# NTV-UIT/MARLLB

Hardware: AMD Instinct MI355X
Metric: env-steps/sec (whole node), 4-server LB env, batch 4k→512k at 1/2/4/8 MI355X (higher is better)
Workload: dtype fp32/int32 (f64 reward); 1 GPU; LB env random-policy rollout, 4 servers (BASELINE configs[1] rollout at the north-star batch); assign_policy=sed, envs_per_gpu=65536, servers=4, global_batch=65536, autoreset=True, autoreset_mode=same_step, parallelism=env-shard x1, dyn_mapping=auto

## Files before the change

### marllb_amd/csrc/lbsim_dyn_group.h

```cpp
#pragma once

#include "lbsim_cross.h"
#include "lbsim_delay.h"
#include "lbsim_kernels.h"
#include "lbsim_workers.h"

namespace lbk {

constexpr int kGroupWL = 8;

template <int CTRL>
__device__ __forceinline__ uint32_t gdpp(uint32_t v) {
  return (uint32_t)__builtin_amdgcn_mov_dpp((int)v, CTRL, 0xF, 0xF, true);
}
__device__ __forceinline__ int32_t f32_key(float x) {
  const int32_t b = (int32_t)__float_as_uint(x);
  return b ^ ((b >> 31) & 0x7FFFFFFF);
}
__device__ __forceinline__ float key_f32(int32_t k) {
  return __uint_as_float((uint32_t)(k ^ ((k >> 31) & 0x7FFFFFFF)));
}
template <int CTRL>
__device__ __forceinline__ void gmin_step(int32_t& a, int32_t& b) {
  const int32_t oa = (int32_t)gdpp<CTRL>((uint32_t)a);
  const int32_t ob = (int32_t)gdpp<CTRL>((uint32_t)b);
  a = oa < a ? oa : a;
  b = ob < b ? ob : b;
}
template <int G>
__device__ __forceinline__ void group_min2(int32_t& a, int32_t& b) {
  gmin_step<0xB1>(a, b);
  if constexpr (G >= 4) gmin_step<0x4E>(a, b);
  if constexpr (G >= 8) gmin_step<0x141>(a, b);
  if constexpr (G >= 16) gmin_step<0x140>(a, b);
  if constexpr (G >= 32) {
    int32_t oa = __shfl_xor(a, 16, 64), ob = __shfl_xor(b, 16, 64);
    a = oa < a ? oa : a;
    b = ob < b ? ob : b;
    if constexpr (G >= 64) {
      oa = __shfl_xor(a, 32, 64);
      ob = __shfl_xor(b, 32, 64);
      a = oa < a ? oa : a;
      b = ob < b ? ob : b;
    }
  }
}
template <int G>
__device__ __forceinline__ int32_t group_min_i32(int32_t v) {
  int32_t o = (int32_t)gdpp<0xB1>((uint32_t)v);
  v = o < v ? o : v;
  if constexpr (G >= 4) { o = (int32_t)gdpp<0x4E>((uint32_t)v); v = o < v ? o : v; }
  if constexpr (G >= 8) { o = (int32_t)gdpp<0x141>((uint32_t)v); v = o < v ? o : v; }
  if constexpr (G >= 16) { o = (int32_t)gdpp<0x140>((uint32_t)v); v = o < v ? o : v; }
  if constexpr (G >= 32) { o = __shfl_xor(v, 16, 64); v = o < v ? o : v; }
  if constexpr (G >= 64) { o = __shfl_xor(v, 32, 64); v = o < v ? o : v; }
  return v;
}
template <int G>
__device__ __forceinline__ uint32_t group_add(uint32_t v) {
  v += gdpp<0xB1>(v);
  if constexpr (G >= 4) v += gdpp<0x4E>(v);
  if constexpr (G >= 8) v += gdpp<0x141>(v);
  if constexpr (G >= 16) v += gdpp<0x140>(v);
  if constexpr (G >= 32) v += (uint32_t)__shfl_xor((int)v, 16, 64);
  if constexpr (G >= 64) v += (uint32_t)__shfl_xor((int)v, 32, 64);
  return v;
}
template <int G>
__device__ __forceinline__ uint32_t group_or(uint32_t v) {
  v |= gdpp<0xB1>(v);
  if constexpr (G >= 4) v |= gdpp<0x4E>(v);
  if constexpr (G >= 8) v |= gdpp<0x141>(v);
  if constexpr (G >= 16) v |= gdpp<0x140>(v);
  if constexpr (G >= 32) v |= (uint32_t)__shfl_xor((int)v, 16, 64);
  if constexpr (G >= 64) v |= (uint32_t)__shfl_xor((int)v, 32, 64);
  return v;
}
template <int G>
__device__ __forceinline__ uint64_t group_bits(uint64_t m, int gbase) {
  return G == 64 ? m : (m >> gbase) & ((1ull << (G & 63)) - 1ull);
}

struct SrvLane {
  int32_t cnt, head_tc, head, lh, tail, last, assigned;
  int32_t qcap;
  bool big;
  uint32_t rcnt;
  int32_t lost;
  uint32_t* chgw;
  float score, scale;
  double den, rcp;
  bool act;
  uint32_t rcnt_d;
  int32_t phead, pcnt;
  uint32_t pdue, over;
  uint32_t* fs_row;
  uint32_t fs_cnt, fs_max;
  unsigned long long fs_sum;
};

__device__ __forceinline__ void flow_stats_add(SrvLane& V, uint32_t fct) {
  if (V.fs_row == nullptr) return;
  V.fs_cnt += 1u;
  V.fs_sum += fct;
  V.fs_max = fct > V.fs_max ? fct : V.fs_max;
  V.fs_row[flow_bin(fct)] += 1u;
}

struct CrossLane {
  bool on = false;
  uint32_t thr = 0u, edge = 0u, salt = 0u;
};

struct WorkLane {
  bool on = false;
  int32_t c = 1;
};

struct DelayLane {
  bool pend = false;
  int32_t r = 0;
  float w2 = 1.0f;
};

struct LaneQueue {
  int2* win;
  int2* ring;
  int lane, lh, head, Q;
  __device__ __forceinline__ int2 get(int pos) const {
    int2 e;
    if (workers_in_window(pos, kGroupWL)) {
      e = win[workers_win_slot(lh, pos, kGroupWL) * 64 + lane];
    } else {
      e = ring[(uint32_t)workers_ring_index(head, pos, Q)];
      asm volatile("");
    }
    return e;
  }
  __device__ __forceinline__ void set(int pos, const int2& e) const {
    if (workers_in_window(pos, kGroupWL)) {
      win[workers_win_slot(lh, pos, kGroupWL) * 64 + lane] = e;
    } else {
      ring[(uint32_t)workers_ring_index(head, pos, Q)] = e;
      asm volatile("");
    }
  }
};

struct GroupAliasTab {
  int32_t* t;
  int gbase;
  __device__ int32_t& operator()(int f, int k) const { return t[f * 64 + gbase + k]; }
};

__device__ __forceinline__ void split_add(const DevState& st, const SimParams& p, SrvLane& V,
                                          uint32_t sb, uint32_t gid, uint32_t episode, int s,
                                          bool is_dur, uint32_t v, uint32_t ts_ms, bool has_r,
                                          uint32_t r) {
  const uint32_t c = is_dur ? V.rcnt_d : V.rcnt;
  const int slot = res_slot(p, c, has_r, r, gid, episode,
                            (kStreamReservoir << 24) | (is_dur ? 0u : 1u << 16) | (uint32_t)s);
  if (slot >= 0) {
    if (!has_r && v >= kPackLimit) V.big = true;
    uint2* rec = is_dur ? reinterpret_cast<uint2*>(st.res_dur) : st.res;
    rec[(size_t)sb * K + (uint32_t)slot] = make_uint2(v, ts_ms);
    atomicOr(V.chgw + ((uint32_t)slot >> 5) * 64u, 1u << (slot & 31));
  }
  if (is_dur) V.rcnt_d = count_inc(c);
  else V.rcnt = count_inc(c);
}
__device__ __forceinline__ void split_flush(const DevState& st, const SimParams& p, SrvLane& V,
                                            uint32_t sb, uint32_t gid, uint32_t episode, int s,
                                            int32_t t, uint64_t base_us) {
  const int P = p.pend_P;
  const uint2* ring = st.pend + (size_t)sb * (uint32_t)P;
  while (V.pcnt > 0) {
    const int32_t rel = (int32_t)(V.pdue - (uint32_t)base_us);
    if (rel > t) break;
    const uint32_t val = ring[V.phead].y;
    const uint32_t ts = (uint32_t)((uint64_t)((int64_t)base_us + (int64_t)rel) / 1000u);
    split_add(st, p, V, sb, gid, episode, s, false, val, ts, false, 0u);
    V.phead = V.phead + 1 == P ? 0 : V.phead + 1;
    V.pcnt -= 1;
    if (V.pcnt > 0) V.pdue = ring[V.phead].x;
  }
}
__device__ __forceinline__ void split_push(const DevState& st, const SimParams& p, SrvLane& V,
                                           uint32_t sb, uint32_t due, uint32_t val) {
  const int P = p.pend_P;
  if (V.pcnt == P) {
    V.over += 1u;
    return;
  }
  uint2* ring = st.pend + (size_t)sb * (uint32_t)P;
  int i = V.pcnt;
  while (i > 0) {
    int pos = V.phead + i - 1;
    pos = pos >= P ? pos - P : pos;
    const uint2 e = ring[pos];
    if ((int32_t)(e.x - due) <= 0) break;
    ring[pos + 1 == P ? 0 : pos + 1] = e;
    --i;
  }
  int pos = V.phead + i;
  pos = pos >= P ? pos - P : pos;
  ring[pos] = make_uint2(due, val);
  V.pcnt += 1;
  if (i == 0) V.pdue = due;
}
__device__ __forceinline__ void split_complete(const DevState& st, const SimParams& p, SrvLane& V,
                                               uint32_t sb, uint32_t gid, uint32_t episode, int s,
                                               int32_t tc, int32_t ta, uint32_t dur, uint32_t ts_ms,
                                               bool has_r, uint32_t r, uint64_t base_us) {
  split_flush(st, p, V, sb, gid, episode, s, tc, base_us);
  split_add(st, p, V, sb, gid, episode, s, true, dur, ts_ms, has_r, r);
  int32_t wait = 0;
  if (lf_wait(p, (uint32_t)base_us + (uint32_t)ta, gid, episode, wait))
    split_push(st, p, V, sb,
               (uint32_t)base_us + (uint32_t)tc + (uint32_t)(p.lf_off_us + 40000000) +
                   (uint32_t)wait,
               lf_guess((uint32_t)(tc - ta), p.lf_off_us, wait));
  else
    split_add(st, p, V, sb, gid, episode, s, false, (uint32_t)(tc - ta), ts_ms, has_r, r);
}
__device__ __forceinline__ void vpp_zero_bins(const DevState& st, const SimParams& p, uint32_t sb) {
  uint4* r4 = reinterpret_cast<uint4*>(st.res + (size_t)sb * K);
  for (int i = 0; i < K / 2; ++i) r4[i] = make_uint4(0u, 0u, 0u, 0u);
  if (st.res_dur != nullptr) {
    const int n4 = p.split ? K / 2 : K / 4;
    uint4* d4 = reinterpret_cast<uint4*>(st.res_dur + (size_t)sb * K * (p.split ? 2u : 1u));
    for (int i = 0; i < n4; ++i) d4[i] = make_uint4(0u, 0u, 0u, 0u);
  }
}

struct GroupConst {
  uint32_t k0, k1;
  float mean_gap;
  int32_t dt;
  uint32_t base_ms, base_rem;
};
__device__ __forceinline__ GroupConst group_const(const SimParams& p, float mean_gap,
                                                  uint32_t base_ms, uint32_t base_rem) {
  GroupConst c;
  c.k0 = vpin(p.key0);
  c.k1 = vpin(p.key1);
  c.mean_gap = vpin(mean_gap);
  c.dt = vpin(p.dt_us);
  c.base_ms = vpin(base_ms);
  c.base_rem = vpin(base_rem);
  return c;
}

template <int G, int POLICY, bool TRACE, bool FAST, bool FULL = false, bool DELAY = false>
__device__ __forceinline__ void group_event_loop(const DevState& st, const SimParams& p,
                                                 LaneState<1>& E, SrvLane& V, int s, int gbase,
                                                 int n_alias, const GroupConst& gc, int2* win,
                                                 int32_t* atab, int4* acache, uint2* const my_res,
                                                 int2* const my_ring, bool fs_on = false,
                                                 const TraceSel& ts = TraceSel{},
                                                 const WorkSel& ws = WorkSel{},
                                                 const CrossLane& cx = CrossLane{},
                                                 const WorkLane& wk = WorkLane{},
                                                 DelayLane dl = DelayLane{}) {
  constexpr int WL = kGroupWL;
  constexpr bool two_choice = (POLICY == 1 || POLICY == 3);
  constexpr bool alias = POLICY == kPolicyAlias;
  constexpr bool lsq = (POLICY == 2 || POLICY == 3);
  const int S = p.S, Q = p.Q;
  const int32_t dt = gc.dt;
  const GroupAliasTab tab{atab, gbase};
  const int lane = gbase + s;
  auto wslot = [&](int i) -> int2* { return win + i * 64 + lane; };
  auto mark = [&](int slot) {
    atomicOr(V.chgw + ((uint32_t)slot >> 5) * 64u, 1u << (slot & 31));
  };
  uint32_t cbase = 0u;
  uint32_t it = 0u;
  uint32_t kbase = E.arr_idx + 1u, rbase = 0u;
  if constexpr (TRACE) rbase = trace_row_in(ts.rows, E.gid, E.episode, kbase);
  for (;;) {
    if constexpr (DELAY && !lsq) {
      if (dl.pend && E.next_arr >= dl.r) {
        dl.pend = false;
        if constexpr (alias) {
          const float w2 = dl.w2;
          n_alias = build_alias_fn<G>([&](int k) { return __shfl(w2, gbase + k, 64); }, S, tab);
        } else if (V.act) {
          V.den = (double)dl.w2 + 1e-9;
          V.rcp = 1.0 / V.den;
        }
      }
    }
    if ((it & (uint32_t)(G - 1)) == 0u) {
      cbase = E.arr_idx + 1u;
      const uint32_t k = cbase + (uint32_t)s;
      uint32_t rk0[10], rk1[10];
      const uint32_t k0 = gc.k0, k1 = gc.k1;
#pragma unroll
      for (int r = 0; r < 10; ++r) {
        rk0[r] = k0 + (uint32_t)r * 0x9E3779B9u;
        rk1[r] = k1 + (uint32_t)r * 0xBB67AE85u;
      }
      const u32x4 d = philox_rk(u32x4{k, E.gid, E.episode, kStreamArrival << 24}, rk0, rk1);
      int32_t gap;
      float wk;
      if constexpr (TRACE) {
        const uint32_t rows = ts.rows;
        rbase += cbase - kbase;
        kbase = cbase;
        while (rbase >= rows) rbase -= rows;
        uint32_t r = rbase + (uint32_t)s;
        while (r >= rows) r -= rows;
        gap = (int32_t)st.trace_gap[ts.base + r];
        wk = st.trace_work[ts.base + r];
      } else if (FULL && ws.tab != nullptr) {
        table_arrival(ws, d.x, d.y, gc.mean_gap, gap, wk);
      } else {
        gap = (int32_t)(-lb_logf(u01_open0(d.x)) * gc.mean_gap);
        wk = -lb_logf(u01_open0(d.y));
      }
      acache[lane] = make_int4(gap, __float_as_int(wk), (int)d.z, (int)d.w);
      __builtin_amdgcn_wave_barrier();
    }
    const int4 nx = acache[gbase + (int)(E.arr_idx + 1u - cbase)];
    ++it;
    const bool arrival_due = E.next_arr < dt;
    const int32_t th = arrival_due ? E.next_arr : dt;
    const bool due = V.act && V.cnt > 0 && V.head_tc <= th;
    if constexpr (FULL) {
      if (cx.on) {
        if (due && wslot(V.lh)->y == kHiddenTa) V.lost += 1;
      } else if (p.leak && due &&
                 lf_lost(p, gc.base_ms * 1000u + gc.base_rem + (uint32_t)wslot(V.lh)->y, E.gid,
                         E.episode)) {
        V.lost += 1;
      }
    }
    if (due && V.cnt > WL) {
      int pw = V.head + WL;
      pw = pw >= Q ? pw - Q : pw;
      *wslot(V.lh) = my_ring[(uint32_t)pw];
      __builtin_amdgcn_s_waitcnt(kWaitVmcnt0);
    }
    const int nl = (V.lh + 1) & (WL - 1);
    const int32_t nt = wslot(nl)->x;
    V.last = due ? V.head_tc : V.last;
    V.cnt -= due ? 1 : 0;
    V.head = due ? ((V.head + 1 == Q) ? 0 : V.head + 1) : V.head;
    V.lh = due ? nl : V.lh;
    V.head_tc = due ? nt : V.head_tc;
    const bool more = group_bits<G>(__ballot(due && V.cnt > 0 && nt <= th), gbase) != 0ull;
    if (!arrival_due && !more) break;
    const bool arr = arrival_due && !more;

    const int32_t ta = E.next_arr;
    if constexpr (!alias) {
      const int32_t nfo = FULL ? V.cnt + V.lost : V.cnt;
      if constexpr (lsq) {
        V.score = (float)nfo;
      } else {
        const double c = (double)(nfo + 1);
        const double q0 = c * V.rcp;
        double q = fma(fma(-q0, V.den, c), V.rcp, q0);
        if (!FAST && q != q) {
          asm volatile("");
          q = c / V.den;
        }
        V.score = (float)q;
      }
    }
    const bool elig = V.act && V.cnt < V.qcap;
    const uint64_t em = group_bits<G>(__ballot(elig), gbase);
    int chosen = -1;
    if constexpr (alias) {
      if (n_alias > 0) {
        const int a = alias_pick(tab, n_alias, E.u2);
        chosen = ((em >> a) & 1u) ? a : -1;
      }
    } else if constexpr (two_choice) {
      const int h1 = two_choice_h1(E.u2, S);
      const int h2 = two_choice_h2(E.u2, S);
      const uint32_t bits = __float_as_uint(V.score);
      const float s1 = __uint_as_float(group_or<G>(s == h1 ? bits : 0u));
      const float s2 = __uint_as_float(group_or<G>(s == h2 ? bits : 0u));
      const bool ok1 = (em >> h1) & 1u, ok2 = (em >> h2) & 1u;
      chosen = (ok1 && ok2) ? ((s2 < s1) ? h2 : h1) : (ok1 ? h1 : (ok2 ? h2 : -1));
    } else if constexpr (FAST) {
      const int32_t key = elig ? f32_key(V.score) : 0x7FFFFFFF;
      const int32_t mk = group_min_i32<G>(key);
      const int h = (int)__umulhi(E.u2, (uint32_t)S);
      const int32_t rk = (elig && key == mk) ? (s == h ? 0 : s + 1) : 0xFF;
      const int32_t mr = group_min_i32<G>(rk);
      chosen = mr == 0xFF ? -1 : (mr == 0 ? h : mr - 1);
    } else {
      const bool num = elig && V.score == V.score;
      const float m = key_f32(group_min_i32<G>(num ? f32_key(V.score) : 0x7f800000));
      const int h = (int)__umulhi(E.u2, (uint32_t)S);
      const int c0 = ((em >> h) & 1u) ? h : (em ? __builtin_ctzll(em) : -1);
      const uint64_t tie = group_bits<G>(__ballot(num && V.score == m), gbase);
      const uint64_t nan = FAST ? 0ull : group_bits<G>(__ballot(V.score != V.score), gbase);
      chosen = c0 < 0 ? -1 : ((((tie | nan) >> c0) & 1u) ? c0 : (tie ? __builtin_ctzll(tie) : -1));
    }
    bool hid = false;
    if constexpr (FULL) {
      if (cx.on) {
        const uint32_t h = cross_hash(E.arr_idx, cx.salt);
        hid = cross_hidden(h, cx.thr);
        const uint32_t x = cross_pick_word(h);
        const int pick =
            __builtin_popcountll(group_bits<G>(__ballot(V.act && cx.edge <= x), gbase));
        chosen = hid ? (((em >> pick) & 1u) ? pick : -1) : chosen;
      }
    }
    const bool push = arr && chosen >= 0;
    E.dropped += (arr && chosen < 0) ? 1u : 0u;
    const bool mine = push && s == chosen;

    int32_t start_a = V.cnt > 0 ? (V.tail > ta ? V.tail : ta) : ta;
    if constexpr (FULL) {
      if (wk.on) {
        if (mine && wk.c > 1)
          start_a = workers_start(LaneQueue{win, my_ring, lane, V.lh, V.head, Q}, V.cnt, wk.c, ta);
      }
    }
    int32_t svc = (int32_t)(E.next_work * V.scale);
    svc = svc < 1 ? 1 : svc;
    const int32_t tc_a = start_a + svc;
    const bool ins = mine && tc_a <= dt;

    int slot = (FULL && p.res_vpp) ? (int)(E.u3 >> 25) : reservoir_slot_r32(V.rcnt, E.u3);
    bool split = false;
    if constexpr (FULL) {
      if (hid) slot = -1;
      if (fs_on && ins && !hid) flow_stats_add(V, (uint32_t)(tc_a - ta));
      split = p.split != 0;
      if (split && ins) {
        const uint64_t base_us = (uint64_t)gc.base_ms * 1000u + gc.base_rem;
        split_complete(st, p, V, (uint32_t)((size_t)(my_res - st.res) / K), E.gid, E.episode, s,
                       tc_a, ta, p.dur_service ? (uint32_t)svc : (uint32_t)(tc_a - ta),
                       gc.base_ms + (gc.base_rem + (uint32_t)tc_a) / 1000u, true, E.u3, base_us);
      }
    }
    if (!split && ins && slot >= 0) {
      const uint32_t fct = (uint32_t)(tc_a - ta);
      my_res[(uint32_t)slot] = make_uint2(fct, gc.base_ms + (gc.base_rem + (uint32_t)tc_a) / 1000u);
      if constexpr (FULL) {
        if (st.res_dur != nullptr)
          st.res_dur[(size_t)(my_res - st.res) + (uint32_t)slot] =
              p.dur_service ? (uint32_t)svc : (uint32_t)(tc_a - ta);
      }
      mark(slot);
    }
    if (mine) {
      const int2 e = make_int2(tc_a, FULL ? (hid ? kHiddenTa : ta) : ta);
      bool sorted = false;
      if constexpr (FULL) {
        if (wk.on) {
          if (wk.c > 1) {
            sorted = true;
            const int at =
                workers_insert(LaneQueue{win, my_ring, lane, V.lh, V.head, Q}, V.cnt, e);
            V.head_tc = at == 0 ? tc_a : V.head_tc;
            V.tail = (V.cnt > 0 && V.tail > tc_a) ? V.tail : tc_a;
          }
        }
      }
      if (!sorted) {
        if (V.cnt < WL) {
          *wslot((V.lh + V.cnt) & (WL - 1)) = e;
        } else {
          int pos = V.head + V.cnt;
          pos = pos >= Q ? pos - Q : pos;
          my_ring[(uint32_t)pos] = e;
          asm volatile("");
        }
        V.tail = tc_a;
      }
      if constexpr (FULL) {
        V.assigned += hid ? 0 : 1;
        V.lost -= hid ? 1 : 0;
      } else {
        V.assigned += 1;
      }
      V.head_tc = V.cnt == 0 ? tc_a : V.head_tc;
      V.cnt += 1;
      if constexpr (FULL) V.rcnt = (ins && !split && !hid) ? count_inc(V.rcnt) : V.rcnt;
      else V.rcnt = (ins && !split) ? count_inc(V.rcnt) : V.rcnt;
    }

    const int32_t na = ta + nx.x;
    const float nw = __int_as_float(nx.y);
    const uint32_t nu2 = (uint32_t)nx.z, nu3 = (uint32_t)nx.w;
    E.next_arr = arr ? na : E.next_arr;
    E.next_work = arr ? nw : E.next_work;
    E.u2 = arr ? nu2 : E.u2;
    E.u3 = arr ? nu3 : E.u3;
    E.arr_idx += arr ? 1u : 0u;
  }
}

template <int G, int POLICY, bool TRACE, bool FULL = false, bool DELAY = false>
__device__ __forceinline__ void sim_step_group(const DevState& st, const SimParams& p,
                                               LaneState<1>& E, SrvLane& V, uint32_t b, int s,
                                               int gbase, float w_own, const float (&wall)[G],
                                               int2* win, int32_t* atab, int4* acache,
                                               bool fs_on = false,
                                               const TraceSel& ts = TraceSel{},
                                               const CrossLane& cx = CrossLane{},
                                               const WorkLane& wk = WorkLane{},
                                               const DelayLane& dl = DelayLane{}) {
  constexpr int WL = kGroupWL;
  const int S = p.S, Q = p.Q;
  const int32_t dt = p.dt_us;
  const uint64_t base_us = (uint64_t)E.clock * (uint64_t)dt;
  const uint32_t base_ms = (uint32_t)(base_us / 1000u);
  const uint32_t base_rem = (uint32_t)(base_us - (uint64_t)base_ms * 1000u);
  constexpr bool alias = POLICY == kPolicyAlias;
  constexpr bool lsq = (POLICY == 2 || POLICY == 3);
  const uint32_t sb = b * (uint32_t)S + (uint32_t)s;
  uint2* const my_res = st.res + (size_t)sb * K;
  int2* const my_ring = st.ring + (size_t)sb * (size_t)Q;
  const GroupAliasTab tab{atab, gbase};
  const int lane = gbase + s;
  int n_alias = 0;
  if constexpr (alias) {
    n_alias = build_alias<G>(wall, S, tab);
  } else if (V.act && !lsq) {
    V.den = (double)w_own + 1e-9;
    V.rcp = 1.0 / V.den;
  }
  auto wslot = [&](int i) -> int2* { return win + i * 64 + lane; };
  auto mark = [&](int slot) {
    atomicOr(V.chgw + ((uint32_t)slot >> 5) * 64u, 1u << (slot & 31));
  };

  if (p.fail_thr != 0u) {
    const u32x4 d = philox4x32_10(
        u32x4{E.clock, E.gid, E.episode, (kStreamFailure << 24) | (uint32_t)s}, p.key0, p.key1);
    const uint32_t u = d.x >> 8;
    const bool was_down = V.qcap == 0;
    const bool fails = V.act && !was_down && u < p.fail_thr;
    const bool recovers = V.act && was_down && u < p.rec_thr;
    E.dropped += group_add<G>(fails ? (uint32_t)V.cnt : 0u);
    if (fails) {
      V.cnt = 0;
      V.last = kLastNone;
      V.rcnt = 0u;
      V.big = false;
      mark(0);
      V.lost = 0;
      if constexpr (FULL) {
        V.rcnt_d = 0u;
        V.pcnt = 0;
        V.phead = 0;
        if (p.res_vpp) vpp_zero_bins(st, p, sb);
      }
    }
    V.qcap = fails ? 0 : (recovers ? Q : V.qcap);
  }

  if (V.act && V.cnt > 0 && V.head_tc <= dt) {
    int32_t prev = V.last;
    uint32_t rc = V.rcnt;
    auto insert = [&](int32_t etc, int32_t eta) {
      if constexpr (FULL) {
        if (eta == kHiddenTa) {
          prev = etc;
          return;
        }
        if (fs_on) flow_stats_add(V, (uint32_t)(etc - eta));
      }
      if (FULL && p.split) {
        split_complete(st, p, V, sb, E.gid, E.episode, s, etc, eta,
                       dur_sample(p, etc, eta, eta > prev ? eta : prev),
                       base_ms + (base_rem + (uint32_t)etc) / 1000u, false, 0u, base_us);
        rc = V.rcnt;
      } else {
        const u32x4 d = philox4x32_10(
            u32x4{rc >> 1, E.gid, E.episode, (kStreamReservoir << 24) | (uint32_t)s}, p.key0,
            p.key1);
        const int slot =
            (FULL && p.res_vpp) ? (int)(((rc & 1u) ? d.w : d.y) >> 25) : reservoir_slot(rc, d);
        if (slot >= 0) {
          const uint32_t fct = (uint32_t)(etc - eta);
          const uint32_t dur = FULL ? dur_sample(p, etc, eta, eta > prev ? eta : prev) : fct;
          V.big |= big_record(fct, dur);
          store_record(st, (size_t)sb * K + (uint32_t)slot, fct, dur,
                       base_ms + (base_rem + (uint32_t)etc) / 1000u);
          mark(slot);
        }
        rc = count_inc(rc);
      }
      prev = etc;
    };
    const int nwin = V.cnt < WL ? V.cnt : WL;
    int i = 0;
    bool past = false;
    for (; i < nwin; ++i) {
      const int2 e = *wslot((V.lh + i) & (WL - 1));
      if (e.x > dt) {
        past = true;
        break;
      }
      insert(e.x, e.y);
    }
    if (!past) {
      int pos = V.head + i;
      pos = pos >= Q ? pos - Q : pos;
      for (; i < V.cnt; ++i) {
        const int2 e = my_ring[(uint32_t)pos];
        if (e.x > dt) break;
        insert(e.x, e.y);
        pos = pos + 1 == Q ? 0 : pos + 1;
      }
    }
    V.rcnt = rc;
  }

  const GroupConst gc = group_const(p, env_mean_gap(st, p, b), base_ms, base_rem);
  WorkSel ws{};
  if constexpr (FULL && !TRACE) ws = env_work_sel(st, b);
  const bool finite = lsq || alias || !V.act ||
                      (fabs(V.den) >= 1e-30 && fabs(V.den) <= 1e300);
  if constexpr (FULL) {
    group_event_loop<G, POLICY, TRACE, false, true, DELAY>(st, p, E, V, s, gbase, n_alias, gc, win,
                                                           atab, acache, my_res, my_ring, fs_on,
                                                           ts, ws, cx, wk, dl);
    if (p.split && V.act) split_flush(st, p, V, sb, E.gid, E.episode, s, dt, base_us);
  } else if (__all(finite)) {
    group_event_loop<G, POLICY, TRACE, true>(st, p, E, V, s, gbase, n_alias, gc, win, atab,
                                             acache, my_res, my_ring, false, ts, ws);
  } else {
    group_event_loop<G, POLICY, TRACE, false>(st, p, E, V, s, gbase, n_alias, gc, win, atab,
                                              acache, my_res, my_ring, false, ts, ws);
  }

  E.next_arr -= dt;
  if (V.act) {
    for (int i = 0; i < WL && i < V.cnt; ++i) {
      int2* e = wslot((V.lh + i) & (WL - 1));
      e->x -= dt;
      if constexpr (FULL) e->y = e->y == kHiddenTa ? kHiddenTa : e->y - dt;
      else e->y -= dt;
    }
    int pos = V.head + WL;
    if (pos >= Q) pos -= Q;
    for (int i = WL; i < V.cnt; ++i) {
      int2 e = my_ring[(uint32_t)pos];
      e.x -= dt;
      if constexpr (FULL) e.y = e.y == kHiddenTa ? kHiddenTa : e.y - dt;
      else e.y -= dt;
      my_ring[(uint32_t)pos] = e;
      pos = (pos + 1 == Q) ? 0 : pos + 1;
    }
    V.head_tc -= dt;
    V.tail -= dt;
    V.last = (V.last < kLastNone + dt) ? kLastNone : V.last - dt;
  }
  E.clock += 1u;
}

template <int POLICY>
struct DynGroupLds {
  int2 win[kGroupWL * 64];
  int4 acache[64];
  uint32_t chgw[4 * 64];
  int32_t atab[POLICY == kPolicyAlias ? 2 * 64 : 1];
};

template <int G, int MODE, int POLICY, bool TRACE, bool FULL = false, bool DELAY = false>
__device__ __forceinline__ void dyn_group_wave(const DevState& st, const SimParams& p,
                                               const void* action, int action_dtype,
                                               int32_t* assign_out, const uint8_t* reset_mask,
                                               uint32_t wave, int lane, DynGroupLds<POLICY>& L,
                                               const FlowStats& fs = FlowStats{},
                                               const CrossTraffic& ct = CrossTraffic{},
                                               const ServerWorkers& sw = ServerWorkers{},
                                               const ActionDelay& ad = ActionDelay{}) {
  static_assert(G == 2 || G == 4 || G == 8 || G == 16 || G == 32 || G == 64,
                "group = a power of two lanes of the wave");
  constexpr int WL = kGroupWL;
  constexpr bool alias = POLICY == kPolicyAlias;
  int2* const win = L.win;
  int32_t* const atab = L.atab;
  int4* const acache = L.acache;
  uint32_t* const chgw = L.chgw;
  const int s = lane & (G - 1);
  const int gbase = lane & ~(G - 1);
  const int epw = p.dyn_epw > 0 ? p.dyn_epw : 64 / G;
  if (lane / G >= epw) return;
  const uint32_t b = wave * (uint32_t)epw + (uint32_t)(lane / G);
  if (b >= (uint32_t)p.B) return;
  const int S = p.S, Q = p.Q;
  if (MODE == kModeReset && reset_mask != nullptr && reset_mask[b] == 0) return;

  LaneState<1> E;
  E.gid = p.env_id_offset + b;
  TraceSel ts{};
  if constexpr (TRACE) ts = env_trace_sel(st, p, b);
  SrvLane V;
  V.act = s < S;
  V.over = 0u;
  uint32_t lfo_base = 0u;
  V.scale = p.svc_scale[0];
#pragma unroll
  for (int k = 1; k < G; ++k) V.scale = (k == s) ? p.svc_scale[k] : V.scale;
  if (st.env_scale != nullptr) V.scale = st.env_scale[b * (uint32_t)S + (uint32_t)(V.act ? s : 0)];
  V.den = 1.0;
  V.rcp = 1.0;
  V.score = 0.f;
  V.assigned = 0;
  V.lh = 0;
#pragma unroll
  for (int w = 0; w < 4; ++w) chgw[w * 64 + lane] = 0u;
  V.chgw = chgw + lane;
  V.fs_row = nullptr;
  V.fs_cnt = 0u;
  V.fs_max = 0u;
  V.fs_sum = 0ull;
  const uint32_t sb = b * (uint32_t)S + (uint32_t)s;
  float wall[G];
  float w_own = 1.0f;
  const bool fs_on = FULL && fs.hist != nullptr;
  CrossLane cx;
  if constexpr (FULL) {
    if (ct.thr != nullptr) {
      cx.on = true;
      cx.thr = ct.thr[b];
      cx.edge = V.act ? ct.cum[sb] : kCrossOne;
    }
  }
  WorkLane wk;
  if constexpr (FULL) {
    if (sw.c != nullptr) {
      wk.on = true;
      wk.c = V.act ? sw.c[sb] : 1;
    }
  }

  auto reset_in = [&]() {
    E.episode = st.episode[b] + 1u;
    E.clock = 0u;
    E.dropped = 0u;
    E.arr_idx = 0u;
    WorkSel ws{};
    if constexpr (FULL && !TRACE) ws = env_work_sel(st, b);
    draw_arrival<1, TRACE>(st, p, E, b, 0, ts, ws);
    V.cnt = 0;
    V.head_tc = 0;
    V.head = 0;
    V.tail = 0;
    V.last = kLastNone;
    V.rcnt = 0u;
    V.qcap = Q;
    V.big = false;
    V.lost = 0;
    V.rcnt_d = 0u;
    V.phead = 0;
    V.pcnt = 0;
    V.pdue = 0u;
    lfo_base = 0u;
    if constexpr (FULL) {
      if (p.res_vpp && V.act) vpp_zero_bins(st, p, sb);
    }
    if (V.act) chgw[lane] = 1u;
#pragma unroll
    for (int k = 0; k < G; ++k) wall[k] = 1.0f;
  };
  auto load_in = [&]() {
    const uint32_t sbl = V.act ? sb : b * (uint32_t)S;
    E.episode = st.episode[b];
    E.clock = st.clock[b];
    E.dropped = st.dropped[b];
    E.arr_idx = st.arr_idx[b];
    E.next_arr = st.next_arr[b];
    E.next_work = st.next_work[b];
    E.u2 = st.next_u2[b];
    E.u3 = st.next_u3[b];
    const uint32_t hc = st.hc[sbl];
    const int32_t last = st.last_tc[sbl];
    const uint32_t rcnt = st.res_count[sbl];
    const float aw = action_weight_sel(p, action, action_dtype, (size_t)sbl);
    V.qcap = Q;
    V.lost = 0;
    V.rcnt_d = 0u;
    V.phead = 0;
    V.pcnt = 0;
    V.pdue = 0u;
    if (FULL && p.split) lfo_base = st.lf_over[b];
    if (FULL && V.act) {
      if (p.leak) V.lost = (int32_t)st.lost_on[sb];
      if constexpr (FULL) {
        if (cx.on) V.lost = (int32_t)st.lost_on[sb];
      }
      if (p.split) {
        V.rcnt_d = st.res_count_dur[sb];
        const uint32_t ph = st.pend_hc[sb];
        V.phead = (int32_t)(ph & 0xFFFFu);
        V.pcnt = (int32_t)(ph >> 16);
        if (V.pcnt > 0) V.pdue = st.pend[(size_t)sb * (uint32_t)p.pend_P + (uint32_t)V.phead].x;
      }
      if (fs.hist != nullptr) {
        V.fs_row = fs.hist + (size_t)sb * kFlowBins;
        V.fs_cnt = fs.count[sb];
        V.fs_max = fs.max_us[sb];
        V.fs_sum = fs.sum[sb];
      }
    }
    if (st.down != nullptr && V.act && st.down[sb] != 0u) V.qcap = 0;
    const int head = V.act ? (int)(hc & kHcHead) : 0;
    const int cnt = V.act ? (int32_t)(hc >> 16) : 0;
    int2 wv[WL];
    const int2* const row = st.ring + sbl * (uint32_t)Q;
#pragma unroll
    for (int i = 0; i < WL; ++i) wv[i] = make_int2(0, 0);
#pragma unroll
    for (int i = 0; i < WL; ++i) {
      if (i < cnt) {
        int pos = head + i;
        pos = pos >= Q ? pos - Q : pos;
        wv[i] = row[pos];
      }
    }
    V.head = head;
    V.big = V.act && (hc & kHcBig) != 0u;
    V.cnt = cnt;
    V.last = V.act ? last : kLastNone;
    V.rcnt = V.act ? rcnt : 0u;
#pragma unroll
    for (int i = 0; i < WL; ++i)
      if (i < cnt) win[i * 64 + lane] = wv[i];
    int32_t tail = wv[0].x;
#pragma unroll
    for (int i = 1; i < WL; ++i) tail = cnt == i + 1 ? wv[i].x : tail;
    if (cnt > WL) {
      int tp = head + cnt - 1;
      if (tp >= Q) tp -= Q;
      tail = row[tp].x;
    }
    V.tail = cnt > 0 ? tail : 0;
    V.head_tc = cnt > 0 ? wv[0].x : 0;
    if (V.act) w_own = aw;
    if constexpr (alias) {
#pragma unroll
      for (int k = 0; k < G; ++k)
        wall[k] = k < S ? action_weight(p, action, action_dtype, (size_t)b * S + (size_t)k) : 1.0f;
    }
  };
  auto reset_out = [&](int32_t ep_step) {
    V.assigned = 0;
    if (s == 0) {
      st.ep_step[b] = ep_step;
      st.ep_return[b] = 0.0;
    }
  };
  auto cross_in = [&]() {
    if constexpr (FULL) {
      if (cx.on) cx.salt = cross_salt(p.key0, p.key1, E.gid, E.episode);
    }
  };
  DelayLane dl;
  auto delay_in = [&]() {
    if constexpr (DELAY) {
      const int32_t k = st.ep_step[b];
      const uint32_t d = ad.delay_us[b];
      const int32_t m = delay_whole(d, p.dt_us), r = delay_rem(d, p.dt_us);
      float* const rows = ad.wring + (size_t)b * (size_t)(ad.R * S) + (size_t)(V.act ? s : 0);
      const float own = w_own;
      auto word = [&](int32_t j) -> float {
        if (delay_is_ones(j) || !V.act) return 1.0f;
        if (j == k) return own;
        return rows[delay_row(j, ad.R) * S];
      };
      const float w_new = word(delay_step_new(k, m));
      const float w_old = word(delay_step_old(k, m));
      if (V.act && k >= 0) rows[delay_row(k, ad.R) * S] = own;
      dl.r = r;
      dl.pend = r != 0;
      dl.w2 = w_new;
      w_own = r != 0 ? w_old : w_new;
      if constexpr (alias) {
#pragma unroll
        for (int j = 0; j < G; ++j) wall[j] = __shfl(w_own, gbase + j, 64);
      }
    }
  };
  if constexpr (MODE == kModeStep) {
    load_in();
    cross_in();
    delay_in();
    sim_step_group<G, POLICY, TRACE, FULL, DELAY>(st, p, E, V, b, s, gbase, w_own, wall, win,
                                                  atab, acache, fs_on, ts, cx, wk, dl);
  } else if constexpr (MODE == kModeReset) {
    reset_in();
    cross_in();
    for (int k = 0; k < p.warmup_steps; ++k)
      sim_step_group<G, POLICY, TRACE, FULL>(st, p, E, V, b, s, gbase, 1.0f, wall, win, atab,
                                             acache, fs_on, ts, cx, wk);
    reset_out(0);
  } else {
    const bool rs = st.ep_step[b] >= p.max_steps;
    if (rs) reset_in();
    else load_in();
    cross_in();
    if constexpr (DELAY) {
      if (!rs) delay_in();
    }
    const int nsteps = rs ? p.warmup_steps : 1;
    const float w = rs ? 1.0f : w_own;
    for (int k = 0; k < nsteps; ++k)
      sim_step_group<G, POLICY, TRACE, FULL, DELAY>(st, p, E, V, b, s, gbase, w, wall, win, atab,
                                                    acache, fs_on, ts, cx, wk, dl);
    if (rs) reset_out(-1);
  }

  if (V.act) {
    for (int i = 0; i < WL && i < V.cnt; ++i) {
      int pos = V.head + i;
      if (pos >= Q) pos -= Q;
      int li = V.lh + i;
      li = li >= WL ? li - WL : li;
      st.ring[sb * (uint32_t)Q + (uint32_t)pos] = win[li * 64 + lane];
    }
    if (p.big_in_step) {
      const uint32_t cw[4] = {chgw[lane], chgw[64 + lane], chgw[128 + lane], chgw[192 + lane]};
      __builtin_amdgcn_s_waitcnt(0);
      __asm__ volatile("" ::: "memory");
      V.big |= big_written(st, sb, cw, V.rcnt, V.rcnt_d);
    }
    if (FULL && p.split) {
      st.res_count_dur[sb] = V.rcnt_d;
      st.pend_hc[sb] = (uint32_t)V.phead | ((uint32_t)V.pcnt << 16);
    }
    st.hc[sb] = (uint32_t)V.head | (V.big ? kHcBig : 0u) | ((uint32_t)V.cnt << 16);
    st.last_tc[sb] = V.last;
    st.res_count[sb] = V.rcnt;
    if (st.down != nullptr) st.down[sb] = V.qcap == 0 ? 1u : 0u;
    if (FULL && (p.leak || cx.on)) st.lost_on[sb] = (uint32_t)V.lost;
    if (FULL && V.fs_row != nullptr) {
      fs.count[sb] = V.fs_cnt;
      fs.max_us[sb] = V.fs_max;
      fs.sum[sb] = V.fs_sum;
    }
    *reinterpret_cast<uint4*>(st.chg + (size_t)sb * 4) =
        make_uint4(chgw[lane], chgw[64 + lane], chgw[128 + lane], chgw[192 + lane]);
    if (MODE != kModeReset && assign_out != nullptr) assign_out[sb] = V.assigned;
  }
  const uint32_t over = (FULL && p.split) ? group_add<G>(V.over) : 0u;
  if (s == 0) {
    if (FULL && p.split) st.lf_over[b] = lfo_base + over;
    st.episode[b] = E.episode;
    st.clock[b] = E.clock;
    st.dropped[b] = E.dropped;
    st.arr_idx[b] = E.arr_idx;
    st.next_arr[b] = E.next_arr;
    st.next_work[b] = E.next_work;
    st.next_u2[b] = E.u2;
    st.next_u3[b] = E.u3;
  }
}

template <int G, int MODE, int POLICY, bool TRACE, int WAVES = 1>
__global__ void __launch_bounds__(64, WAVES)
    dynamics_group_kernel(DevState st, SimParams p, const void* action, int action_dtype,
                          int32_t* assign_out, const uint8_t* reset_mask) {
  __shared__ DynGroupLds<POLICY> L;
  dyn_group_wave<G, MODE, POLICY, TRACE>(st, p, action, action_dtype, assign_out, reset_mask,
                                         blockIdx.x, (int)threadIdx.x, L);
}

template <int G, int MODE, int POLICY, bool TRACE>
__global__ void __launch_bounds__(64)
    dynamics_group_full_kernel(DevState st, SimParams p, const void* action, int action_dtype,
                               int32_t* assign_out, const uint8_t* reset_mask, FlowStats fs,
                               CrossTraffic ct, ServerWorkers sw) {
  __shared__ DynGroupLds<POLICY> L;
  dyn_group_wave<G, MODE, POLICY, TRACE, true>(st, p, action, action_dtype, assign_out,
                                               reset_mask, blockIdx.x, (int)threadIdx.x, L, fs, ct,
                                               sw);
}

template <int G, int MODE, int POLICY, bool TRACE>
__global__ void __launch_bounds__(64)
    dynamics_group_delay_kernel(DevState st, SimParams p, const void* action, int action_dtype,
                                int32_t* assign_out, const uint8_t* reset_mask, FlowStats fs,
                                CrossTraffic ct, ServerWorkers sw, ActionDelay ad) {
  static_assert(MODE != kModeReset, "a reset has no delay");
  __shared__ DynGroupLds<POLICY> L;
  dyn_group_wave<G, MODE, POLICY, TRACE, true, true>(st, p, action, action_dtype, assign_out,
                                                     reset_mask, blockIdx.x, (int)threadIdx.x, L,
                                                     fs, ct, sw, ad);
}

}
```

Baseline: 303.8 million env-steps/s.

## Add count-based group event loop for non-full groups larger than two

Adds a new per-arrival loop that works out each server's queue length by counting window entries whose completion time is past the arrival time. It refills the window from the ring buffer on demand, instead of running the event loop that retires completions one by one. The head, tail and last-completion state are rebuilt once the loop ends, and failure and head-completion handling are adjusted to keep the tail and last values consistent. The aim is to cut per-event work and divergence in the SED policy path, at the cost of a scan of the window on every arrival and extra ring loads with waitcnt stalls.

```diff
diff --git a/marllb_amd/csrc/lbsim_dyn_group.h b/marllb_amd/csrc/lbsim_dyn_group.h
--- a/marllb_amd/csrc/lbsim_dyn_group.h
+++ b/marllb_amd/csrc/lbsim_dyn_group.h
@@ -499,6 +499,192 @@
   }
 }
 
+constexpr int32_t kGroupFree = -(1 << 30);
+
+template <int G, int POLICY, bool TRACE, bool FAST>
+__device__ __forceinline__ void group_count_loop(const DevState& st, const SimParams& p,
+                                                 LaneState<1>& E, SrvLane& V, int s, int gbase,
+                                                 int n_alias, const GroupConst& gc, int2* win,
+                                                 int32_t* atab, int4* acache, uint2* const my_res,
+                                                 int2* const my_ring,
+                                                 const TraceSel& ts = TraceSel{}) {
+  constexpr int WL = kGroupWL;
+  constexpr bool two_choice = (POLICY == 1 || POLICY == 3);
+  constexpr bool alias = POLICY == kPolicyAlias;
+  constexpr bool lsq = (POLICY == 2 || POLICY == 3);
+  const int S = p.S, Q = p.Q;
+  const int32_t dt = gc.dt;
+  const GroupAliasTab tab{atab, gbase};
+  const int lane = gbase + s;
+  auto wslot = [&](int i) -> int2* { return win + i * 64 + lane; };
+  auto mark = [&](int slot) {
+    atomicOr(V.chgw + ((uint32_t)slot >> 5) * 64u, 1u << (slot & 31));
+  };
+  const int nw0 = V.cnt < WL ? V.cnt : WL;
+#pragma unroll
+  for (int i = 0; i < WL; ++i)
+    if (i >= nw0) wslot((V.lh + i) & (WL - 1))->x = kGroupFree;
+  int nring = V.cnt - nw0;
+  int wpos = (V.lh + nw0) & (WL - 1);
+  int pidx = V.head + V.cnt;
+  pidx = pidx >= Q ? pidx - Q : pidx;
+  int32_t lastdone = V.last;
+  auto count_at = [&](int32_t t) -> int {
+    int n_win = 0;
+#pragma unroll
+    for (int k = 0; k < WL; ++k) n_win += wslot(k)->x > t ? 1 : 0;
+    while (nring > 0 && n_win < WL) {
+      int ri = pidx - nring;
+      ri = ri < 0 ? ri + Q : ri;
+      const int2 e = my_ring[(uint32_t)ri];
+      __builtin_amdgcn_s_waitcnt(kWaitVmcnt0);
+      *wslot(wpos) = e;
+      wpos = (wpos + 1) & (WL - 1);
+      nring -= 1;
+      n_win += e.x > t ? 1 : 0;
+    }
+    return n_win;
+  };
+  uint32_t cbase = 0u;
+  uint32_t it = 0u;
+  uint32_t kbase = E.arr_idx + 1u, rbase = 0u;
+  if constexpr (TRACE) rbase = trace_row_in(ts.rows, E.gid, E.episode, kbase);
+  int n_end;
+  for (;;) {
+    const bool arrival = E.next_arr < dt;
+    const int32_t ta = arrival ? E.next_arr : dt;
+    const int n_win = count_at(ta);
+    if (!arrival) {
+      n_end = n_win;
+      break;
+    }
+    if ((it & (uint32_t)(G - 1)) == 0u) {
+      cbase = E.arr_idx + 1u;
+      const uint32_t k = cbase + (uint32_t)s;
+      uint32_t rk0[10], rk1[10];
+      const uint32_t k0 = gc.k0, k1 = gc.k1;
+#pragma unroll
+      for (int r = 0; r < 10; ++r) {
+        rk0[r] = k0 + (uint32_t)r * 0x9E3779B9u;
+        rk1[r] = k1 + (uint32_t)r * 0xBB67AE85u;
+      }
+      const u32x4 d = philox_rk(u32x4{k, E.gid, E.episode, kStreamArrival << 24}, rk0, rk1);
+      int32_t gap;
+      float wk;
+      if constexpr (TRACE) {
+        const uint32_t rows = ts.rows;
+        rbase += cbase - kbase;
+        kbase = cbase;
+        while (rbase >= rows) rbase -= rows;
+        uint32_t r = rbase + (uint32_t)s;
+        while (r >= rows) r -= rows;
+        gap = (int32_t)st.trace_gap[ts.base + r];
+        wk = st.trace_work[ts.base + r];
+      } else {
+        gap = (int32_t)(-lb_logf(u01_open0(d.x)) * gc.mean_gap);
+        wk = -lb_logf(u01_open0(d.y));
+      }
+      acache[lane] = make_int4(gap, __float_as_int(wk), (int)d.z, (int)d.w);
+      __builtin_amdgcn_wave_barrier();
+    }
+    const int4 nx = acache[gbase + (int)(E.arr_idx + 1u - cbase)];
+    ++it;
+    const int n = n_win + nring;
+
+    if constexpr (!alias) {
+      if constexpr (lsq) {
+        V.score = (float)n;
+      } else {
+        const double c = (double)(n + 1);
+        const double q0 = c * V.rcp;
+        double q = fma(fma(-q0, V.den, c), V.rcp, q0);
+        if (!FAST && q != q) {
+          asm volatile("");
+          q = c / V.den;
+        }
+        V.score = (float)q;
+      }
+    }
+    const bool elig = V.act && n < V.qcap;
+    int chosen = -1;
+    if constexpr (alias) {
+      const uint64_t em = group_bits<G>(__ballot(elig), gbase);
+      if (n_alias > 0) {
+        const int a = alias_pick(tab, n_alias, E.u2);
+        chosen = ((em >> a) & 1u) ? a : -1;
+      }
+    } else if constexpr (two_choice) {
+      const uint64_t em = group_bits<G>(__ballot(elig), gbase);
+      const int h1 = two_choice_h1(E.u2, S);
+      const int h2 = two_choice_h2(E.u2, S);
+      const uint32_t bits = __float_as_uint(V.score);
+      const float s1 = __uint_as_float(group_or<G>(s == h1 ? bits : 0u));
+      const float s2 = __uint_as_float(group_or<G>(s == h2 ? bits : 0u));
+      const bool ok1 = (em >> h1) & 1u, ok2 = (em >> h2) & 1u;
+      chosen = (ok1 && ok2) ? ((s2 < s1) ? h2 : h1) : (ok1 ? h1 : (ok2 ? h2 : -1));
+    } else if constexpr (FAST) {
+      const int32_t key = elig ? f32_key(V.score) : 0x7FFFFFFF;
+      const int32_t mk = group_min_i32<G>(key);
+      const int h = (int)__umulhi(E.u2, (uint32_t)S);
+      const int32_t rk = (elig && key == mk) ? (s == h ? 0 : s + 1) : 0xFF;
+      const int32_t mr = group_min_i32<G>(rk);
+      chosen = mr == 0xFF ? -1 : (mr == 0 ? h : mr - 1);
+    } else {
+      const uint64_t em = group_bits<G>(__ballot(elig), gbase);
+      const bool num = elig && V.score == V.score;
+      const float m = key_f32(group_min_i32<G>(num ? f32_key(V.score) : 0x7f800000));
+      const int h = (int)__umulhi(E.u2, (uint32_t)S);
+      const int c0 = ((em >> h) & 1u) ? h : (em ? __builtin_ctzll(em) : -1);
+      const uint64_t tie = group_bits<G>(__ballot(num && V.score == m), gbase);
+      const uint64_t nan = group_bits<G>(__ballot(V.score != V.score), gbase);
+      chosen = c0 < 0 ? -1 : ((((tie | nan) >> c0) & 1u) ? c0 : (tie ? __builtin_ctzll(tie) : -1));
+    }
+    E.dropped += chosen < 0 ? 1u : 0u;
+    const bool mine = s == chosen;
+
+    const int32_t start_a = V.tail > ta ? V.tail : ta;
+    int32_t svc = (int32_t)(E.next_work * V.scale);
+    svc = svc < 1 ? 1 : svc;
+    const int32_t tc_a = start_a + svc;
+    const bool ins = mine && tc_a <= dt;
+
+    const int slot = reservoir_slot_r32(V.rcnt, E.u3);
+    if (ins && slot >= 0) {
+      const uint32_t fct = (uint32_t)(tc_a - ta);
+      my_res[(uint32_t)slot] = make_uint2(fct, gc.base_ms + (gc.base_rem + (uint32_t)tc_a) / 1000u);
+      mark(slot);
+    }
+    if (mine) {
+      const int2 e = make_int2(tc_a, ta);
+      if (n_win < WL) {
+        *wslot(wpos) = e;
+        wpos = (wpos + 1) & (WL - 1);
+      } else {
+        my_ring[(uint32_t)pidx] = e;
+        asm volatile("");
+        nring += 1;
+      }
+      pidx = pidx + 1 == Q ? 0 : pidx + 1;
+      V.tail = tc_a;
+      V.assigned += 1;
+      V.rcnt = ins ? count_inc(V.rcnt) : V.rcnt;
+      lastdone = ins ? tc_a : lastdone;
+    }
+
+    E.next_arr = ta + nx.x;
+    E.next_work = __int_as_float(nx.y);
+    E.u2 = (uint32_t)nx.z;
+    E.u3 = (uint32_t)nx.w;
+    E.arr_idx += 1u;
+  }
+  V.cnt = n_end + nring;
+  int head = pidx - V.cnt;
+  V.head = head < 0 ? head + Q : head;
+  V.lh = (wpos - n_end) & (WL - 1);
+  V.head_tc = V.cnt > 0 ? wslot(V.lh)->x : V.head_tc;
+  V.last = lastdone;
+}
+
 template <int G, int POLICY, bool TRACE, bool FULL = false, bool DELAY = false>
 __device__ __forceinline__ void sim_step_group(const DevState& st, const SimParams& p,
                                                LaneState<1>& E, SrvLane& V, uint32_t b, int s,
@@ -517,6 +703,7 @@
   const uint32_t base_rem = (uint32_t)(base_us - (uint64_t)base_ms * 1000u);
   constexpr bool alias = POLICY == kPolicyAlias;
   constexpr bool lsq = (POLICY == 2 || POLICY == 3);
+  constexpr bool COUNT = !FULL && G > 2;
   const uint32_t sb = b * (uint32_t)S + (uint32_t)s;
   uint2* const my_res = st.res + (size_t)sb * K;
   int2* const my_ring = st.ring + (size_t)sb * (size_t)Q;
@@ -544,6 +731,7 @@
     E.dropped += group_add<G>(fails ? (uint32_t)V.cnt : 0u);
     if (fails) {
       V.cnt = 0;
+      if constexpr (COUNT) V.tail = 0;
       V.last = kLastNone;
       V.rcnt = 0u;
       V.big = false;
@@ -615,6 +803,7 @@
       }
     }
     V.rcnt = rc;
+    if constexpr (COUNT) V.last = prev;
   }
 
   const GroupConst gc = group_const(p, env_mean_gap(st, p, b), base_ms, base_rem);
@@ -627,12 +816,19 @@
                                                            atab, acache, my_res, my_ring, fs_on,
                                                            ts, ws, cx, wk, dl);
     if (p.split && V.act) split_flush(st, p, V, sb, E.gid, E.episode, s, dt, base_us);
+  } else if constexpr (!COUNT) {
+    if (__all(finite))
+      group_event_loop<G, POLICY, TRACE, true>(st, p, E, V, s, gbase, n_alias, gc, win, atab,
+                                               acache, my_res, my_ring, false, ts, ws);
+    else
+      group_event_loop<G, POLICY, TRACE, false>(st, p, E, V, s, gbase, n_alias, gc, win, atab,
+                                                acache, my_res, my_ring, false, ts, ws);
   } else if (__all(finite)) {
-    group_event_loop<G, POLICY, TRACE, true>(st, p, E, V, s, gbase, n_alias, gc, win, atab,
-                                             acache, my_res, my_ring, false, ts, ws);
+    group_count_loop<G, POLICY, TRACE, true>(st, p, E, V, s, gbase, n_alias, gc, win, atab,
+                                             acache, my_res, my_ring, ts);
   } else {
-    group_event_loop<G, POLICY, TRACE, false>(st, p, E, V, s, gbase, n_alias, gc, win, atab,
-                                              acache, my_res, my_ring, false, ts, ws);
+    group_count_loop<G, POLICY, TRACE, false>(st, p, E, V, s, gbase, n_alias, gc, win, atab,
+                                              acache, my_res, my_ring, ts);
   }
 
   E.next_arr -= dt;
```

Result: faster. 325.1 million env-steps/s (median of 6 runs) (+7.0%).
